# Youssef-Harby/flac-raster

Measured on AMD Instinct MI355X. Metric: Mpixels/sec encode (create-streaming) + bbox-extract ms, 1/2/4/8 GPU; bit-exact vs ref, higher is better.
Workload: dtype int16; 1 GPU; C4 create-streaming encode (band 1, device-resident); raster=40000x40000x4 int16, tile_size=512, tiles=6241, tiles_rank0=6241, blocksize=4096, compression_level=5, parallelism=single GPU (no exchange), compressed_bytes_rank0=3134407161, compressed_bytes_total=3134407161

## Files before the change

flac_raster_amd/csrc/frs_encode.hip:

```cpp

#include <type_traits>

#include <cstring>
#include <unistd.h>

#include "frs_internal.h"
#include "frs_frame_header.h"

namespace frs {

template <int DT> struct Elem;
template <> struct Elem<FRS_DT_U8> { using T = uint8_t; static constexpr bool is_float = false; };
template <> struct Elem<FRS_DT_U16> { using T = uint16_t; static constexpr bool is_float = false; };
template <> struct Elem<FRS_DT_I16> { using T = int16_t; static constexpr bool is_float = false; };
template <> struct Elem<FRS_DT_I32> { using T = int32_t; static constexpr bool is_float = false; };
template <> struct Elem<FRS_DT_U32> { using T = uint32_t; static constexpr bool is_float = false; };
template <> struct Elem<FRS_DT_F32> { using T = float; static constexpr bool is_float = true; };
template <> struct Elem<FRS_DT_F64> { using T = double; static constexpr bool is_float = true; };

__device__ inline int64_t f2key(double v) {
    int64_t b = __double_as_longlong(v);
    return b >= 0 ? b : (b ^ 0x7FFFFFFFFFFFFFFFll);
}
__host__ __device__ inline double key2f(int64_t k) {
    int64_t b = k >= 0 ? k : (k ^ 0x7FFFFFFFFFFFFFFFll);
    double d;
    memcpy(&d, &b, 8);
    return d;
}

template <int DT> __device__ inline int64_t elem_key(typename Elem<DT>::T v) {
    if constexpr (Elem<DT>::is_float) return f2key((double)v);
    else return (int64_t)v;
}

template <int DT> __device__ inline int32_t spatial_norm(typename Elem<DT>::T x) {
    if constexpr (DT == FRS_DT_U8) return cast_f64_i32_x86((double)__fdiv_rn(__fsub_rn((float)x, 127.5f), 127.5f));
    else if constexpr (DT == FRS_DT_U16) return cast_f64_i32_x86((double)__fdiv_rn(__fsub_rn((float)x, 32767.5f), 32767.5f));
    else if constexpr (DT == FRS_DT_I16) return cast_f64_i32_x86((double)__fdiv_rn((float)x, 32767.0f));
    else if constexpr (DT == FRS_DT_I32) return cast_f64_i32_x86((double)__fdiv_rn((float)x, 2147483647.0f));
    else if constexpr (DT == FRS_DT_F32) return cast_f64_i32_x86((double)fminf(fmaxf(x, -1.0f), 1.0f));
    else return 0;
}

template <int DT> struct Normalizer {
    using T = typename Elem<DT>::T;
    T mn;
    double den;
    double rinv;
    double scale;
    int has_range;
    int bps16;
    int spatial;
    int fastdiv;
    __device__ inline int32_t operator()(T x) const {
        if (spatial) return spatial_norm<DT>(x);
        if constexpr (DT == FRS_DT_F32) {
            float v = x * 8388607.0f;
            return cast_f64_i32_x86((double)v);
        } else if constexpr (DT == FRS_DT_F64) {
            return cast_f64_i32_x86(x * 8388607.0);
        } else {
            if (!has_range) return 0;
            T d = (T)((int64_t)x - (int64_t)mn);
            double v;
            if (fastdiv) {
                const double a = 2.0 * (double)d;
                const double q0 = a * rinv;
                v = fma(fma(-q0, den, a), rinv, q0) - 1.0;
            } else {
                v = (2.0 * (double)d) / den - 1.0;
            }
            v = v * scale;
            int32_t c = cast_f64_i32_x86(v);
            return bps16 ? (int32_t)(int16_t)c : c;
        }
    }
};

template <int DT> __device__ inline Normalizer<DT> make_norm(const TileNorm &tn, int scale_bits, int norm_mode) {
    Normalizer<DT> nz;
    nz.spatial = norm_mode == 1;
    using T = typename Elem<DT>::T;
    if constexpr (!Elem<DT>::is_float) nz.mn = (T)tn.imin;
    else nz.mn = (T)0;
    nz.den = tn.den;
    nz.rinv = tn.rinv;
    nz.fastdiv = tn.mode == kNormLut || tn.mode == kNormFastDiv;
    nz.scale = scale_bits == 16 ? 32767.0 : 8388607.0;
    nz.has_range = tn.has_range;
// ... 1277 lines not shown
            __syncthreads();
            uint64_t wbase = 0;
            for (int k = 0; k < wv; k++) wbase += wtot[k];
            const uint64_t excl = wbase + incl - my;
            uint64_t total = 0;
            for (int k = 0; k < kEncThreads / 64; k++) total += wtot[k];
            sub_end = pos + (uint64_t)pbits * (1 << po) + total;
            if (sub_end > (uint64_t)kWords * 32 - 64) {
                if (tid == 0) atomicOr(error_flag, 2);
                return;
            }
            uint64_t run = excl;
            __shared__ uint64_t pstart[1 << kMaxPo];
            for (int i = max(i_beg, o); i < i_end; i++) {
                const int32_t r32 = (int32_t)resid(Lc, type == 2, o, i);
                const uint32_t u = ((uint32_t)r32 << 1) ^ (uint32_t)(r32 >> 31);
                const int p = i / ps;
                const int k = rc.k[p];
                const uint32_t q = u >> k;
                const int first_of_p = p == 0 ? o : p * ps;
                if (i == first_of_p) pstart[p] = run;
                const uint64_t at = pos + (uint64_t)pbits * (p + 1) + run + q;
                const uint32_t low = k ? (u & ((1u << k) - 1u)) : 0u;
                put_bits(S.bits, at, (1u << k) | low, k + 1);
                run += 1 + (uint64_t)k + q;
            }
            __syncthreads();
            for (int p = tid; p < (1 << po); p += kEncThreads)
                put_bits(S.bits, pos + (uint64_t)pbits * p + pstart[p], rc.k[p], pbits);
            }
        }
        __syncthreads();
        {
            const uint64_t full = sub_end >> 5;
            if ((int64_t)(w0 + full) + 2 > P.slot_words) {
                if (tid == 0) atomicOr(error_flag, 1);
                return;
            }
            for (uint64_t i = tid; i < full; i += kEncThreads) slot[w0 + i] = __builtin_bswap32(S.bits[i]);
            __syncthreads();
            const uint32_t keep = S.bits[full];
            __syncthreads();
            for (int i = tid; i < kWords; i += kEncThreads) S.bits[i] = 0;
            __syncthreads();
            if (tid == 0) S.bits[0] = keep;
            __syncthreads();
            w0 += (int64_t)full;
            fb = sub_end - (full << 5);
        }
    }
    const uint64_t bits_total = (uint64_t)w0 * 32 + fb;
    const uint64_t bytes = (bits_total + 7) >> 3;
    if (fb && tid == 0) slot[w0] = __builtin_bswap32(S.bits[0]);
    if (tid == 0) frame_bytes[si] = (int64_t)bytes + 2;
}

__constant__ uint16_t c_crc16[256];
__constant__ uint16_t c_xpow8[40];

__device__ inline uint32_t gf_mulmod(uint32_t a, uint32_t b) {
    uint32_t r = 0;
#pragma unroll
    for (int i = 15; i >= 0; i--) {
        r <<= 1;
        if (r & 0x10000u) r ^= 0x18005u;
        if ((b >> i) & 1u) r ^= a;
    }
    return r;
}

__device__ inline uint32_t xpow8(uint64_t m) {
    uint32_t r = 1;
    int j = 0;
    while (m) {
        if (m & 1) r = gf_mulmod(r, c_xpow8[j]);
        m >>= 1;
        j++;
    }
    return r;
}

constexpr int kFrameWordsV3 = 2176;
constexpr int kXpowBytes = kFrameWordsV3 * 4 + 64;
__constant__ uint16_t c_crc16x8[16][256];
__device__ uint16_t g_xpow_bytes[kXpowBytes];
__device__ uint16_t g_xpow_8k[32];
__device__ inline uint32_t xpow_bytes(int64_t m) {
    if (m < kXpowBytes) return g_xpow_bytes[m];
    if (m < 32 * 8192) return gf_mulmod(g_xpow_bytes[m & 8191], g_xpow_8k[m >> 13]);
    return xpow8((uint64_t)m);
}

__device__ inline uint32_t wg_crc16(const uint8_t *src, int64_t L, const uint16_t (*T)[256], uint32_t *wc) {
    const uint32_t *sw = reinterpret_cast<const uint32_t *>(src);
    const int64_t nw = L >> 2;
    const int64_t ch = (nw + 255) / 256;
    const int64_t w0 = min(nw, (int64_t)threadIdx.x * ch), w1 = min(nw, w0 + ch);
    uint32_t c = 0;
    for (int64_t i = w0; i < w1; i++) {
        const uint32_t v = sw[i];
        c = (uint32_t)T[3][((c >> 8) ^ v) & 0xFF] ^ T[2][((c & 0xFF) ^ (v >> 8)) & 0xFF] ^ T[1][(v >> 16) & 0xFF] ^
            T[0][v >> 24];
    }
    int64_t end = w1 << 2;
    const bool last = (nw == 0) ? threadIdx.x == 0 : (w1 == nw && w1 > w0);
    if (last) {
        for (int64_t i = nw << 2; i < L; i++) c = ((c << 8) & 0xFFFFu) ^ T[0][((c >> 8) ^ src[i]) & 0xFF];
        end = L;
    }
    const int64_t m = L - end;
    if (c && m > 0) c = gf_mulmod(c, xpow_bytes(m));
    for (int o = 32; o > 0; o >>= 1) c ^= __shfl_xor(c, o);
    if ((threadIdx.x & 63) == 0) wc[threadIdx.x >> 6] = c;
    __syncthreads();
    return wc[0] ^ wc[1] ^ wc[2] ^ wc[3];
}

__device__ inline void wg_load_crc_tables(uint16_t (*T)[256]) {
    for (int i = threadIdx.x; i < 1024; i += blockDim.x) (&T[0][0])[i] = (&c_crc16x8[0][0])[i];
    __syncthreads();
}

__global__ void __launch_bounds__(256) k_compact(const uint32_t *slots, int slot_words, const int64_t *frame_bytes,
                                                const int64_t *frame_off, int64_t nframes, uint8_t *arena) {
    __shared__ uint16_t T[4][256];
    __shared__ uint32_t wc[4];
    const int64_t f = blockIdx.x;
    if (f >= nframes) return;
    wg_load_crc_tables(T);
    const uint32_t *sw = slots + (size_t)f * slot_words;
    const uint8_t *src = reinterpret_cast<const uint8_t *>(sw);
    const int64_t S = frame_bytes[f];
    const int64_t L = S - 2;
    uint8_t *dst = arena + frame_off[f];
    const int h = (int)((4 - (reinterpret_cast<uintptr_t>(dst) & 3)) & 3);
    const int64_t hb = min((int64_t)h, L);
    if ((int64_t)threadIdx.x < hb) dst[threadIdx.x] = src[threadIdx.x];
    const int64_t nbw = (L - hb) >> 2;
    uint32_t *dw = reinterpret_cast<uint32_t *>(dst + hb);
    const int sh = (int)(hb & 3);
    const int64_t swords = slot_words;
    for (int64_t k = threadIdx.x; k < nbw; k += 256) {
        const int64_t sbyte = hb + 4 * k, si = sbyte >> 2;
        const uint32_t lo = sw[si], hi = (sh && si + 1 < swords) ? sw[si + 1] : 0u;
        dw[k] = __builtin_amdgcn_alignbyte(hi, lo, (uint32_t)sh);
    }
    for (int64_t i = hb + 4 * nbw + threadIdx.x; i < L; i += 256) dst[i] = src[i];
    const uint32_t crc = wg_crc16(src, L, T, wc);
    if (threadIdx.x == 0) {
        dst[L] = (uint8_t)(crc >> 8);
        dst[L + 1] = (uint8_t)crc;
    }
}

__global__ void __launch_bounds__(256) k_seal_partial(uint32_t *slots, int slot_words, const int64_t *frame_bytes,
                                                     int64_t nlist) {
    __shared__ uint16_t T[4][256];
    __shared__ uint32_t wc[4];
    const int64_t si = blockIdx.x;
    if (si >= nlist) return;
    wg_load_crc_tables(T);
    uint8_t *src = reinterpret_cast<uint8_t *>(slots + (size_t)si * slot_words);
    const int64_t L = frame_bytes[si] - 2;
    const uint32_t crc = wg_crc16(src, L, T, wc);
    if (threadIdx.x == 0) {
        src[L] = (uint8_t)(crc >> 8);
        src[L + 1] = (uint8_t)crc;
    }
}
// ... 737 lines not shown
    v += bfly_partner64<32>(v);
    return ((uint64_t)uni((uint32_t)(v >> 32)) << 32) | uni((uint32_t)v);
}
__device__ inline uint32_t dpp_wave_or_u32(uint32_t v) {
    v |= bfly_partner<1>(v);
    v |= bfly_partner<2>(v);
    v |= bfly_partner<4>(v);
    v |= bfly_partner<8>(v);
    v |= bfly_partner<16>(v);
    v |= bfly_partner<32>(v);
    return uni(v);
}
__device__ inline uint32_t dpp_wave_max_u32(uint32_t v) {
    v = max(v, bfly_partner<1>(v));
    v = max(v, bfly_partner<2>(v));
    v = max(v, bfly_partner<4>(v));
    v = max(v, bfly_partner<8>(v));
    v = max(v, bfly_partner<16>(v));
    v = max(v, bfly_partner<32>(v));
    return uni(v);
}
__device__ inline uint32_t dpp_wave_xor_u32(uint32_t v) {
    v ^= bfly_partner<1>(v);
    v ^= bfly_partner<2>(v);
    v ^= bfly_partner<4>(v);
    v ^= bfly_partner<8>(v);
    v ^= bfly_partner<16>(v);
    v ^= bfly_partner<32>(v);
    return uni(v);
}
__device__ inline uint32_t dpp_incl_scan_u32(uint32_t v) {
    v += (uint32_t)__builtin_amdgcn_update_dpp(0, (int)v, 0x111, 0xF, 0xF, false);
    v += (uint32_t)__builtin_amdgcn_update_dpp(0, (int)v, 0x112, 0xF, 0xF, false);
    v += (uint32_t)__builtin_amdgcn_update_dpp(0, (int)v, 0x114, 0xF, 0xF, false);
    v += (uint32_t)__builtin_amdgcn_update_dpp(0, (int)v, 0x118, 0xF, 0xF, false);
    v += (uint32_t)__builtin_amdgcn_update_dpp(0, (int)v, 0x142, 0xA, 0xF, false);
    v += (uint32_t)__builtin_amdgcn_update_dpp(0, (int)v, 0x143, 0xC, 0xF, false);
    return v;
}
__device__ inline uint32_t dpp_wave_shr1(uint32_t v) {
    return (uint32_t)__builtin_amdgcn_update_dpp(0, (int)v, 0x138, 0xF, 0xF, false);
}

typedef short v2s16 __attribute__((ext_vector_type(2)));
__device__ inline int32_t dot2(uint32_t a, uint32_t b, int32_t c) {
    return __builtin_amdgcn_sdot2(__builtin_bit_cast(v2s16, a), __builtin_bit_cast(v2s16, b), c, false);
}
__device__ inline uint32_t pack2(int32_t lo, int32_t hi) { return ((uint32_t)lo & 0xFFFFu) | ((uint32_t)hi << 16); }

__device__ inline int32_t dot2_z(uint32_t a, uint32_t b) {
    int32_t d;
    asm("v_dot2_i32_i16 %0, %1, %2, 0" : "=v"(d) : "v"(a), "v"(b));
    return d;
}

__device__ inline void residual_pair(const uint32_t *E, const uint32_t *C, int shift, int m, int32_t &re, int32_t &ro) {
    const int b = 4 + m;
    const uint32_t o0 = __builtin_amdgcn_perm(E[b], E[b - 1], 0x05040302u);
    const uint32_t o1 = __builtin_amdgcn_perm(E[b - 1], E[b - 2], 0x05040302u);
    const uint32_t o2 = __builtin_amdgcn_perm(E[b - 2], E[b - 3], 0x05040302u);
    const uint32_t o3 = __builtin_amdgcn_perm(E[b - 3], E[b - 4], 0x05040302u);
    int32_t se = dot2_z(E[b - 1], C[0]);
    int32_t so = dot2_z(o0, C[0]);
    se = dot2(E[b - 2], C[1], se);
    so = dot2(o1, C[1], so);
    se = dot2(E[b - 3], C[2], se);
    so = dot2(o2, C[2], so);
    se = dot2(E[b - 4], C[3], se);
    so = dot2(o3, C[3], so);
    const uint32_t v = E[b];
    re = (int32_t)(int16_t)(v & 0xFFFFu) - (se >> shift);
    ro = ((int32_t)v >> 16) - (so >> shift);
}

constexpr uint64_t kFlagAgg = 1ull << 62, kFlagIncl = 2ull << 62, kValMask = (1ull << 62) - 1;


constexpr int kXpowHi = (kXpowBytes + 63) / 64;
constexpr int kBufWordsV3 = kFrameWordsV3 + 64;
constexpr int kSubWords = kFrameWordsV3 + 4;
struct EncV3Shared {
    uint32_t bits[4][kBufWordsV3];
    int16_t lut[kLutCap];
    uint16_t crc8x[16][256];
    uint16_t xlo[64];
    uint16_t xhi[kXpowHi];
    uint8_t crc8[256];
    int ticket[2];
    int want[2];
    int lut_tile;
};
static_assert(offsetof(EncV3Shared, lut) + sizeof(int16_t) * kLutCap <= 65536, "LUT beyond 64 KiB of LDS");

struct FbMap {
    uint32_t c, magic, k;
    __device__ inline uint32_t col(uint32_t w) const { return __umul24(w, magic) >> 20; }
    __device__ inline uint32_t operator()(uint32_t w) const {
        return (uint32_t)__mul24((int)col(w), -(int)k) + (w << 6);
    }
};
__device__ inline FbMap fb_map(uint32_t words) {
    const uint32_t c = max(1u, (words + 63) >> 6);
    return FbMap{c, ((1u << 20) + c - 1) / c, 64 * c - 1};
}
__device__ inline void fb_fold(uint32_t *buf, const FbMap &M, int lane) {
    uint32_t *ovr = buf + (M.c << 6) + lane;
    const uint32_t v = *ovr;
    *ovr = 0;
    if (lane < 63 && v) atomicOr(buf + lane + 1, v);
}

__device__ inline void lds_put_bits2(uint32_t *buf, const FbMap &M, uint32_t pos, uint32_t val, int nbits) {
    const uint32_t wi = pos >> 5;
    const uint64_t v = (uint64_t)val << (64 - (int)(pos & 31) - nbits);
    atomicOr(&buf[M(wi)], (uint32_t)(v >> 32));
    atomicOr(&buf[M(wi + 1)], (uint32_t)v);
}

__device__ inline void reg_fence(uint32_t *E) {
#pragma unroll
    for (int m = 0; m < 36; m++) asm volatile("" : "+v"(E[m]));
}

__device__ inline uint32_t sad_u32(uint32_t a, uint32_t b, uint32_t c) {
    uint32_t d;
    asm("v_sad_u32 %0, %1, %2, %3" : "=v"(d) : "v"(a), "v"(b), "v"(c));
    return d;
}

__device__ inline void lds_put_left(uint32_t *buf, const FbMap &M, int nk4, uint32_t pos, uint32_t codeL) {
    const uint32_t hi = __builtin_amdgcn_alignbit(0u, codeL, pos);
    const uint32_t lo = __builtin_amdgcn_alignbit(codeL, 0u, pos);
    const uint32_t wi = pos >> 5;
    uint32_t *p = reinterpret_cast<uint32_t *>(reinterpret_cast<char *>(buf) + (wi << 8) +
                                               __mul24((int)M.col(wi), nk4));
    atomicOr(p, hi);
    atomicOr(p + 64, lo);
}

__device__ inline void lut_gather_pairs(const uint32_t *w, const int16_t *lut, int32_t imin, uint32_t *out) {
    const uint32_t lb = (uint32_t)reinterpret_cast<uintptr_t>(lut);
    const uint32_t c16 = (lb - 2u * (uint32_t)imin) & 0xFFFFu, cc = c16 | (c16 << 16), two = 0x00020002u;
    const char *lds0 = reinterpret_cast<const char *>(lut) - lb;
#pragma unroll
    for (int m = 0; m < 32; m++) {
        uint32_t a;
        asm("v_pk_mad_u16 %0, %1, %2, %3" : "=v"(a) : "v"(w[m]), "v"(two), "v"(cc));
        const uint32_t lo = *reinterpret_cast<const uint16_t *>(lds0 + (a & 0xFFFFu));
        const uint32_t hi = *reinterpret_cast<const uint16_t *>(lds0 + (a >> 16));
        out[m] = lo | (hi << 16);
    }
}

__device__ inline uint32_t zigzag(int32_t r) { return ((uint32_t)r << 1) ^ (uint32_t)(r >> 31); }

struct PendingFrame {
    int64_t f = -1;
    uint64_t fbytes = 0;
    bool ok = true;
    FbMap map{1, 1u << 20, 63};
};

__device__ __forceinline__ void resolve_and_store(const EncodeParams &P, PendingFrame &pf, uint32_t *fbuf, uint8_t *arena,
                                         int64_t arena_cap, int64_t *frame_off, uint64_t *status, int *err, int lane) {
    const int64_t f = pf.f;
    const uint64_t fbytes = pf.fbytes;
    const bool ok = pf.ok;
    const bool l0 = lane == 0;
    uint64_t prefix = 0;
// ... 330 lines not shown
                uint32_t k = (g[c] < 2 || prod == 0) ? 0u : 32u - (uint32_t)__builtin_clz(prod);
                k = min(k, 14u);
                Kp[c] |= k << (4 * (5 - po));
                V[c][5 - po] = 4 + (1 + k) * ns + ((2 * g[c]) >> k) - (ns >> 1);
            }
        }
#pragma unroll
        for (int c = 0; c < NC; c++) V[c][0] += bfly_partner<2>(V[c][0]);
#pragma unroll
        for (int c = 0; c < NC; c++)
#pragma unroll
            for (int i = 0; i <= 1; i++) V[c][i] += bfly_partner<4>(V[c][i]);
#pragma unroll
        for (int c = 0; c < NC; c++)
#pragma unroll
            for (int i = 0; i <= 2; i++) V[c][i] += bfly_partner<8>(V[c][i]);
#pragma unroll
        for (int c = 0; c < NC; c++)
#pragma unroll
            for (int i = 0; i <= 3; i++) V[c][i] += bfly_partner<16>(V[c][i]);
#pragma unroll
        for (int c = 0; c < NC; c++)
#pragma unroll
            for (int i = 0; i <= 4; i++) V[c][i] += bfly_partner<32>(V[c][i]);
#pragma unroll
        for (int c = 0; c < NC; c++) {
            uint32_t best_bits = 0;
            int best_i = 0;
#pragma unroll
            for (int i = 0; i < 6; i++) {
                const uint32_t bits = 6 + uni(V[c][i]);
                if (best_bits == 0 || bits < best_bits) {
                    best_bits = bits;
                    best_i = i;
                }
            }
            bb[c] = best_bits;
            bp[c] = 5 - best_i;
            bk[c] = (int)((Kp[c] >> (4 * best_i)) & 15u);
        }
    };
    auto rice = [&](uint32_t lane_sum, int order, uint32_t &best_bits, int &best_po, int &my_k) {
        if (__ballot(lane_sum >= (1u << 24)) == 0) {
            const uint32_t sm[1] = {lane_sum};
            const int od[1] = {order};
            uint32_t b1[1];
            int p1[1], k1[1];
            rice32m(std::integral_constant<int, 1>{}, sm, od, b1, p1, k1);
            best_bits = b1[0], best_po = p1[0], my_k = k1[0];
        } else {
            rice64(lane_sum, order, best_bits, best_po, my_k);
        }
    };
    rb_f = rb_l = 0;
    po_f = po_l = k_f = k_l = 0;
    if (cand_fixed && cand_lpc && __ballot(sf >= (1u << 24) || sl >= (1u << 24)) == 0) {
        uint32_t bb[2];
        int bp[2], bk[2];
        const uint32_t sm[2] = {sf, sl};
        const int od[2] = {of, ol};
        rice32m(std::integral_constant<int, 2>{}, sm, od, bb, bp, bk);
        rb_f = bb[0], po_f = bp[0], k_f = bk[0];
        rb_l = bb[1], po_l = bp[1], k_l = bk[1];
    } else {
        if (cand_fixed) rice(sf, of, rb_f, po_f, k_f);
        if (cand_lpc) rice(sl, ol, rb_l, po_l, k_l);
    }
}

constexpr int kPrivRows = 34;
constexpr uint32_t kPrivBits = kPrivRows * 32;
static_assert(kBufWordsV3 >= (kPrivRows + 1) * 64, "private rows + the spill row");
static_assert(kBufWordsV3 % 4 == 0, "b128 zeroing");

__device__ inline void zero_wave_buf(uint32_t *buf, int lane) {
    uint4 *b4 = reinterpret_cast<uint4 *>(buf);
#pragma unroll
    for (int i = 0; i < (kBufWordsV3 / 4 + 63) / 64; i++) {
        const int c = lane + 64 * i;
        if (i < kBufWordsV3 / 256 || c < kBufWordsV3 / 4) b4[c] = make_uint4(0u, 0u, 0u, 0u);
    }
}

__device__ __forceinline__ uint32_t crc16_cols(const uint32_t *fbuf, const FbMap &M, uint32_t body, const EncV3Shared &S,
                                               int lane) {
    const uint32_t nfw = body >> 2, tail = body & 3;
    const uint32_t wb = min(nfw, (uint32_t)lane * M.c), we = min(nfw, wb + M.c);
    uint32_t c = 0;
    const uint32_t *colp = fbuf + lane;
    const uint16_t(*T)[256] = S.crc8x;
    uint32_t i = wb;
    for (; i + 3 < we; i += 4, colp += 256) {
        const uint32_t w0 = colp[0], w1 = colp[64], w2 = colp[128], w3 = colp[192];
        c = (uint32_t)T[15][((c >> 8) ^ (w0 >> 24)) & 0xFF] ^ T[14][((c & 0xFF) ^ (w0 >> 16)) & 0xFF] ^
            T[13][(w0 >> 8) & 0xFF] ^ T[12][w0 & 0xFF] ^ T[11][w1 >> 24] ^ T[10][(w1 >> 16) & 0xFF] ^
            T[9][(w1 >> 8) & 0xFF] ^ T[8][w1 & 0xFF] ^ T[7][w2 >> 24] ^ T[6][(w2 >> 16) & 0xFF] ^
            T[5][(w2 >> 8) & 0xFF] ^ T[4][w2 & 0xFF] ^ T[3][w3 >> 24] ^ T[2][(w3 >> 16) & 0xFF] ^
            T[1][(w3 >> 8) & 0xFF] ^ T[0][w3 & 0xFF];
    }
    for (; i + 1 < we; i += 2, colp += 128) {
        const uint32_t w0 = colp[0], w1 = colp[64];
        c = (uint32_t)T[7][((c >> 8) ^ (w0 >> 24)) & 0xFF] ^ T[6][((c & 0xFF) ^ (w0 >> 16)) & 0xFF] ^
            T[5][(w0 >> 8) & 0xFF] ^ T[4][w0 & 0xFF] ^ T[3][w1 >> 24] ^ T[2][(w1 >> 16) & 0xFF] ^
            T[1][(w1 >> 8) & 0xFF] ^ T[0][w1 & 0xFF];
    }
    if (i < we) {
        const uint32_t word = *colp;
        c = (uint32_t)T[3][((c >> 8) ^ (word >> 24)) & 0xFF] ^ T[2][((c & 0xFF) ^ (word >> 16)) & 0xFF] ^
            T[1][(word >> 8) & 0xFF] ^ T[0][word & 0xFF];
    }
    uint32_t end = we * 4;
    if (lane == (int)M.col(nfw - 1)) {
        const uint32_t word = fbuf[M(nfw)];
        for (uint32_t b = 0; b < tail; b++) {
            const uint32_t byte = (word >> (24 - 8 * b)) & 0xFF;
            c = ((c << 8) & 0xFFFFu) ^ S.crc8x[0][((c >> 8) ^ byte) & 0xFF];
        }
        end += tail;
    }
    const uint32_t m = body - end;
    return dpp_wave_xor_u32(gf_mulmod(gf_mulmod(c, S.xlo[m & 63]), S.xhi[m >> 6]));
}

template <int DT, bool SUB = false, bool ST = false, bool WIDE = false>
__device__ __forceinline__ void encode_frame_v4(const typename Elem<DT>::T *raster, const EncodeParams &P,
                                                const TileGeom *__restrict__ tiles,
                                                const TileNorm *__restrict__ norms,
                                                const SubAnalysis *__restrict__ ana, uint8_t *arena, int64_t arena_cap,
                                                int64_t *frame_off, uint64_t *status, int *err, EncV3Shared &S,
                                                int want, int64_t f, int lane, const int32_t *ftile,
                                                PendingFrame &prev, const uint4 *hdr_tab, int hdr_n,
                                                const uint32_t *pslots, const int64_t *pbytes, int chn = 0,
                                                uint32_t *sub_slots = nullptr, int32_t *sub_bits = nullptr,
                                                int32_t *sub_est = nullptr) {
    using T = typename Elem<DT>::T;
    using Lane = std::conditional_t<WIDE, LaneWide, LanePairs>;
    uint32_t *fbuf = S.bits[uni_if<!WIDE>(threadIdx.x >> 6)];
    const int t = ftile[f];
    const TileGeom g = tiles[t];
    const bool l0 = lane == 0;
    if (!SUB && g.partial && f - g.frame_base == g.nframes - 1) {
        const int64_t si = g.partial - 1;
        const uint64_t nb = (uint64_t)pbytes[si];
        const uint32_t words = (uint32_t)((nb + 3) >> 2);
        const bool ok = words + 2 <= (uint32_t)kFrameWordsV3;
        if (!ok && l0) atomicOr(err, 2);
        const uint64_t fbytes = ok ? nb : 0;
        const FbMap M = fb_map(words + 1);
        __builtin_amdgcn_s_setprio(2);
        if (l0)
            __hip_atomic_store(&status[f], (f == 0 ? kFlagIncl : kFlagAgg) | fbytes, __ATOMIC_RELAXED,
                               __HIP_MEMORY_SCOPE_AGENT);
        if (prev.f >= 0) resolve_and_store(P, prev, fbuf, arena, arena_cap, frame_off, status, err, lane);
        if (ok) {
            const uint32_t *src = pslots + (size_t)si * P.slot_words;
            for (uint32_t w = (uint32_t)lane; w < words; w += 64) fbuf[M(w)] = __builtin_bswap32(src[w]);
        }
        __builtin_amdgcn_s_waitcnt(0xC07F);
        __builtin_amdgcn_wave_barrier();
        __builtin_amdgcn_s_setprio(0);
        prev.f = f, prev.fbytes = fbytes, prev.ok = ok, prev.map = M;
        return;
    }
    TileNorm tn = norms[t];
    if (t != want && tn.mode == kNormLut) tn.mode = kNormSlow;
    const int16_t *lut = S.lut;
    __builtin_amdgcn_s_setprio(2);
    const int64_t fk = f - g.frame_base;
    const int64_t s0 = fk * kMaxBlock;
    constexpr int n = kMaxBlock;
    const int64_t sub = SUB ? f * P.nvch + chn : f;
    const SubAnalysis A = ana[sub];
    const int w = A.wasted;
    const int sbps = 16 - w + ((ST && chn == 3) ? 1 : 0);
    const T *base = raster + (int64_t)(P.band0 + ((ST && chn >= 2) ? 0 : chn)) * P.band_stride + g.r0 * P.row_stride +
                    g.c0;

    auto load_lane = [&](Lane &Ls) __attribute__((always_inline)) {
        Chunk64<DT> ch;
        const uint32_t sl0 = (uint32_t)s0 + 64u * (uint32_t)lane;
        const uint32_t row = udiv_inv(sl0, (uint32_t)g.w, 1.0 / (double)g.w);
        const int col = (int)(sl0 - row * (uint32_t)g.w), vec = (g.w % 64) == 0 ? P.vec_ok : 0;
        ch.load(base, P.row_stride, g.w, row, col, vec, 64);
        const bool lutp = sizeof(T) == 2 && tn.mode == kNormLut && w == 0;
        auto sx = [](uint32_t v, int h) -> int32_t { return h ? ((int32_t)v >> 16) : (int32_t)(int16_t)(v & 0xFFFFu); };
        if constexpr (WIDE) {
            if (lutp) {
                uint32_t Lp[32], Rp[32];
                lut_gather_pairs(ch.w, lut, (int32_t)tn.imin, Lp);
                ch.load(base + P.band_stride, P.row_stride, g.w, row, col, vec, 64);
                lut_gather_pairs(ch.w, lut, (int32_t)tn.imin, Rp);
#pragma unroll
                for (int m = 0; m < 32; m++) {
                    Ls.X[8 + 2 * m] = sx(Lp[m], 0) - sx(Rp[m], 0);
                    Ls.X[9 + 2 * m] = sx(Lp[m], 1) - sx(Rp[m], 1);
                }
            } else {
                norm_chunk<DT>(ch, tn, lut, [&](int j, int32_t x) { Ls.X[8 + j] = x; });
                ch.load(base + P.band_stride, P.row_stride, g.w, row, col, vec, 64);
                norm_chunk<DT>(ch, tn, lut, [&](int j, int32_t x) { Ls.X[8 + j] = (Ls.X[8 + j] - x) >> w; });
            }
        } else {
            auto pairs = [&](uint32_t *dst, int sh) __attribute__((always_inline)) {
// ... 296 lines not shown
            const int sr = P.sample_rate;
            put8(0xFF);
            put8(0xF8);
            put8((uint32_t)((12 << 4) | src));
            put8((uint32_t)(4 << 1));
            const uint32_t v = (uint32_t)fk;
            if (v < 0x80) put8(v);
            else if (v < 0x800) { put8(0xC0 | (v >> 6)); put8(0x80 | (v & 0x3F)); }
            else if (v < 0x10000) { put8(0xE0 | (v >> 12)); put8(0x80 | ((v >> 6) & 0x3F)); put8(0x80 | (v & 0x3F)); }
            else if (v < 0x200000) { put8(0xF0 | (v >> 18)); put8(0x80 | ((v >> 12) & 0x3F)); put8(0x80 | ((v >> 6) & 0x3F)); put8(0x80 | (v & 0x3F)); }
            else if (v < 0x4000000) { put8(0xF8 | (v >> 24)); put8(0x80 | ((v >> 18) & 0x3F)); put8(0x80 | ((v >> 12) & 0x3F)); put8(0x80 | ((v >> 6) & 0x3F)); put8(0x80 | (v & 0x3F)); }
            else { put8(0xFC | (v >> 30)); put8(0x80 | ((v >> 24) & 0x3F)); put8(0x80 | ((v >> 18) & 0x3F)); put8(0x80 | ((v >> 12) & 0x3F)); put8(0x80 | ((v >> 6) & 0x3F)); put8(0x80 | (v & 0x3F)); }
            if (srx == 12) put8((uint32_t)(sr / 1000));
            else if (srx == 13) { put8((uint32_t)(sr >> 8) & 0xFF); put8((uint32_t)sr & 0xFF); }
            else if (srx == 14) { put8((uint32_t)((sr / 10) >> 8) & 0xFF); put8((uint32_t)(sr / 10) & 0xFF); }
            put8(c8);
        }
        const int typecode = type == 0 ? 0 : type == 1 ? 1 : type == 2 ? 8 + of : 32 + ol - 1;
        lds_put_bits2(fbuf, M, hdr_bits, (uint32_t)(typecode << 1) | (w ? 1u : 0u), 8);
        if (w) lds_put_bits2(fbuf, M, hdr_bits + 8 + (uint32_t)(w - 1), 1, 1);
        if (type == 0) lds_put_bits2(fbuf, M, pos0, xi & ((1u << sbps) - 1u), sbps);
        if (type >= 2) {
            uint32_t qq = pos0 + (uint32_t)o * sbps;
            if (type == 3) {
                lds_put_bits2(fbuf, M, qq, (uint32_t)(A.lpc_prec - 1), 4);
                lds_put_bits2(fbuf, M, qq + 4, (uint32_t)lshift & 31u, 5);
                qq += 9 + (uint32_t)o * A.lpc_prec;
            }
            lds_put_bits2(fbuf, M, qq, (uint32_t)po, 6);
        }
    }
    if (type >= 2) {
        const int i = lane & 7;
        const int32_t qi = ana[sub].q[i];
        const bool warm = lane < 8 && i < o, coef = type == 3 && lane >= 8 && lane < 16 && i < o;
        if (warm) lds_put_bits2(fbuf, M, pos0 + (uint32_t)i * sbps, xi & ((1u << sbps) - 1u), sbps);
        if (coef)
            lds_put_bits2(fbuf, M, pos0 + (uint32_t)o * sbps + 9 + (uint32_t)i * A.lpc_prec,
                          (uint32_t)qi & ((1u << A.lpc_prec) - 1u), A.lpc_prec);
    }
    __builtin_amdgcn_s_waitcnt(0xC07F);
    __builtin_amdgcn_wave_barrier();
    if (fold) {
        fb_fold(fbuf, M, lane);
        __builtin_amdgcn_s_waitcnt(0xC07F);
        __builtin_amdgcn_wave_barrier();
    }
    if constexpr (SUB) {
        if (ok) {
            uint32_t *dst = sub_slots + (size_t)sub * kSubWords;
            const uint32_t nw = (end_bits + 31) >> 5;
            for (uint32_t wi = (uint32_t)lane; wi < nw; wi += 64) dst[wi] = fbuf[M(wi)];
            for (uint32_t i = 0; i < M.c; i++) fbuf[(i << 6) | (uint32_t)lane] = 0;
        } else {
            zero_wave_buf(fbuf, lane);
        }
        if (l0) sub_bits[sub] = ok ? (int32_t)end_bits : -1;
        if (l0 && sub_est) sub_est[sub] = (int32_t)best;
        (void)fbytes;
        return;
    }
    if (ok) {
        const uint32_t crc = crc16_cols(fbuf, M, body, S, lane);
        if (l0) lds_put_bits2(fbuf, M, body << 3, crc, 16);
        __builtin_amdgcn_s_waitcnt(0xC07F);
        __builtin_amdgcn_wave_barrier();
    }
    prev.f = f, prev.fbytes = fbytes, prev.ok = ok, prev.map = M;
}

template <int DT, bool SUB = false, bool ST = false, bool WIDE = false>
__global__ void __launch_bounds__(256, sizeof(typename Elem<DT>::T) <= 2 ? (ST ? 2 : 3) : 1) k_encode_v4(const typename Elem<DT>::T *raster, EncodeParams P,
                                                  const TileGeom *__restrict__ tiles,
                                                  const TileNorm *__restrict__ norms, const int16_t *__restrict__ luts,
                                                  const SubAnalysis *__restrict__ ana, uint8_t *arena, int64_t arena_cap,
                                                  int64_t *frame_off, uint64_t *status, int *ticket_ctr, int *err,
                                                  const int32_t *__restrict__ ftile, const uint4 *__restrict__ hdr_tab,
                                                  int hdr_n, const uint32_t *__restrict__ pslots,
                                                  const int64_t *__restrict__ pbytes, uint32_t *sub_slots = nullptr,
                                                  int32_t *sub_bits = nullptr, int32_t *sub_est = nullptr) {
    __shared__ __attribute__((aligned(16))) EncV3Shared S;
    constexpr bool kUni = !WIDE;
    const int wave = (int)uni_if<kUni>(threadIdx.x >> 6), lane = threadIdx.x & 63;
    for (int i = threadIdx.x; i < 4096; i += blockDim.x) (&S.crc8x[0][0])[i] = (&c_crc16x8[0][0])[i];
    for (int i = threadIdx.x; i < 256; i += blockDim.x) S.crc8[i] = c_crc8[i];
    for (int i = threadIdx.x; i < 64; i += blockDim.x) S.xlo[i] = g_xpow_bytes[i];
    for (int i = threadIdx.x; i < kXpowHi; i += blockDim.x) S.xhi[i] = g_xpow_bytes[64 * i];
    for (int i = threadIdx.x; i < 4 * kBufWordsV3; i += blockDim.x) (&S.bits[0][0])[i] = 0;
    if (threadIdx.x == 0) S.lut_tile = -1;
    PendingFrame prev;
    uint32_t *fbuf = S.bits[wave];
    int it = 0;
    while (true) {
        const int sl = it & 1;
        it++;
        constexpr int kUpfSt = WIDE ? 1 : 3;
        const int upf = ST ? kUpfSt : P.nch;
        const int64_t nunits = SUB ? P.nframes * upf : P.nframes;
        if (threadIdx.x == 0) {
            const int tk = atomicAdd(ticket_ctr, 1);
            S.ticket[sl] = tk;
            const int64_t u0 = (int64_t)tk * 4;
            S.want[sl] = (u0 < nunits) ? ftile[SUB ? u0 / upf : u0] : -1;
        }
        __syncthreads();
        const int64_t fbase = (int64_t)(int)uni_if<kUni>((uint32_t)S.ticket[sl]) * 4;
        if (fbase >= nunits) break;
        const int want = (int)uni_if<kUni>((uint32_t)S.want[sl]);
        if (want != (int)uni_if<kUni>((uint32_t)S.lut_tile)) {
            const TileNorm tw = norms[want];
            if (tw.mode == kNormLut) {
                const int64_t R = min(tw.imax - tw.imin, (int64_t)kLutCap - 1);
                const int16_t *src = luts + (int64_t)want * kLutCap;
                for (int64_t d = threadIdx.x; d <= R; d += blockDim.x) S.lut[d] = src[d];
            }
            __syncthreads();
            if (threadIdx.x == 0) S.lut_tile = want;
        }
        if constexpr (SUB) {
            const int64_t v = fbase + wave;
            if (v < nunits) {
                const int64_t f = v / upf;
                const int chn = WIDE ? 3 : (int)(v - f * upf);
                const TileGeom g = tiles[ftile[f]];
                if (!(g.partial && f - g.frame_base == g.nframes - 1))
                    encode_frame_v4<DT, true, ST, WIDE>(raster, P, tiles, norms, ana, arena, arena_cap, frame_off,
                                                        status, err, S, want, f, lane, ftile, prev, hdr_tab, hdr_n,
                                                        pslots, pbytes, chn, sub_slots, sub_bits, sub_est);
            }
        } else {
            const int64_t f = fbase + wave;
            if (f < nunits)
                encode_frame_v4<DT>(raster, P, tiles, norms, ana, arena, arena_cap, frame_off, status, err, S, want, f,
                                    lane, ftile, prev, hdr_tab, hdr_n, pslots, pbytes);
        }
    }
    if constexpr (!SUB)
        if (prev.f >= 0) resolve_and_store(P, prev, fbuf, arena, arena_cap, frame_off, status, err, lane);
}


__device__ inline int mc_frame_header(uint8_t *h, uint32_t v, int chcode, int sr) {
    return frame_header(h, 4096, sr, 16, chcode, v, c_crc8);
}

__device__ inline int st_pick(const int32_t *est4) {
    const uint32_t e0 = (uint32_t)est4[0], e1 = (uint32_t)est4[1], e2 = (uint32_t)est4[2], e3 = (uint32_t)est4[3];
    const uint32_t bits[4] = {e0 + e1, e0 + e3, e1 + e3, e2 + e3};
    int ca = 0;
    for (int k = 1; k < 4; k++)
        if (bits[k] < bits[ca]) ca = k;
    return ca;
}
__device__ inline void st_subs(int ca, int &a, int &b) {
    a = ca == 2 ? 3 : ca == 3 ? 2 : 0;
    b = ca == 0 ? 1 : ca == 2 ? 1 : 3;
}

__global__ void k_mc_frame_bytes(const EncodeParams P, const TileGeom *tiles, const int32_t *ftile,
                                 const int32_t *sub_bits, const int64_t *pbytes, int64_t *frame_bytes, int *err,
                                 const int32_t *sub_est = nullptr, int8_t *pick = nullptr) {
    const int64_t f = (int64_t)blockIdx.x * blockDim.x + threadIdx.x;
    if (f >= P.nframes) return;
    const TileGeom g = tiles[ftile[f]];
    const int64_t fk = f - g.frame_base;
    if (g.partial && fk == g.nframes - 1) {
        frame_bytes[f] = pbytes[g.partial - 1];
        return;
    }
    uint8_t h[16];
// ... 98 lines not shown
                c = ((c << 8) & 0xFFFFu) ^ T[0][((c >> 8) ^ byte) & 0xFF];
            }
            end = B;
        }
        const int64_t m = B - end;
        if (c && m > 0) c = gf_mulmod(c, xpow_bytes(m));
        for (int d = 32; d > 0; d >>= 1) c ^= __shfl_xor(c, d);
        if ((tid & 63) == 0) wc[tid >> 6] = c;
        __syncthreads();
        const uint32_t crc = wc[0] ^ wc[1] ^ wc[2] ^ wc[3];
        if (tid == 0) {
            W[B >> 2] |= ((crc >> 8) & 0xFF) << (24 - 8 * (B & 3));
            W[(B + 1) >> 2] |= (crc & 0xFF) << (24 - 8 * ((B + 1) & 3));
        }
        __syncthreads();
    }
    const int64_t S = B + 2;
    const int hh = (int)((4 - (reinterpret_cast<uintptr_t>(dst) & 3)) & 3);
    const int64_t hbytes = min((int64_t)hh, S);
    auto byte_at = [&](int64_t i) -> uint8_t { return (uint8_t)(W[i >> 2] >> (24 - 8 * (i & 3))); };
    if (tid < hbytes) dst[tid] = byte_at(tid);
    const int64_t nbw = (S - hbytes) >> 2;
    uint32_t *dw = reinterpret_cast<uint32_t *>(dst + hbytes);
    const int sh = (int)(hbytes & 3);
    for (int64_t k = tid; k < nbw; k += 256) {
        const int64_t si = (hbytes + 4 * k) >> 2;
        const uint32_t lo = __builtin_bswap32(W[si]), hi = sh ? __builtin_bswap32(W[si + 1]) : 0u;
        dw[k] = __builtin_amdgcn_alignbyte(hi, lo, (uint32_t)sh);
    }
    for (int64_t i = hbytes + 4 * nbw + tid; i < S; i += 256) dst[i] = byte_at(i);
}

__global__ void k_fast_finish(const int64_t *frame_off, const uint64_t *status, const TileGeom *tiles,
                              const TileNorm *norms, const int *err_flag, int ntiles, int64_t nframes, int64_t *pack) {
    int t = blockIdx.x * blockDim.x + threadIdx.x;
    double *mm = reinterpret_cast<double *>(pack + ntiles + 1);
    if (t < ntiles) {
        pack[t] = frame_off[tiles[t].frame_base];
        mm[2 * t] = norms[t].dmin;
        mm[2 * t + 1] = norms[t].dmax;
    }
    if (t == ntiles) {
        pack[t] = (int64_t)(status[nframes - 1] & kValMask);
        pack[3 * (int64_t)ntiles + 1] = *err_flag;
    }
}

static bool g_tables_ready[64];

static const uint8_t *host_crc8() {
    static uint8_t t[256];
    static const bool ready = (crc8_table(t), true);
    (void)ready;
    return t;
}

static int upload_tables(frs_ctx *ctx) {
    if (g_tables_ready[ctx->device]) return FRS_OK;
    const uint8_t *t8 = host_crc8();
    uint16_t t16[256];
    for (int i = 0; i < 256; i++) {
        uint16_t d = (uint16_t)(i << 8);
        for (int k = 0; k < 8; k++) d = (d & 0x8000) ? (uint16_t)((d << 1) ^ 0x8005) : (uint16_t)(d << 1);
        t16[i] = d;
    }
    uint16_t xp[40];
    auto mulmod = [](uint32_t a, uint32_t b) {
        uint32_t r = 0;
        for (int i = 15; i >= 0; i--) {
            r <<= 1;
            if (r & 0x10000u) r ^= 0x18005u;
            if ((b >> i) & 1u) r ^= a;
        }
        return r;
    };
    uint32_t v = 0x100;
    for (int j = 0; j < 40; j++) {
        xp[j] = (uint16_t)v;
        v = mulmod(v, v);
    }
    FRS_HIP(hipMemcpyToSymbolAsync(HIP_SYMBOL(c_crc8), t8, 256, 0, hipMemcpyHostToDevice, ctx->stream));
    FRS_HIP(hipMemcpyToSymbolAsync(HIP_SYMBOL(c_crc16), t16, sizeof(t16), 0, hipMemcpyHostToDevice, ctx->stream));
    FRS_HIP(hipMemcpyToSymbolAsync(HIP_SYMBOL(c_xpow8), xp, sizeof(xp), 0, hipMemcpyHostToDevice, ctx->stream));
    static uint16_t t4[16][256];
    static uint16_t xb[kXpowBytes];
    for (int i = 0; i < 256; i++) t4[0][i] = t16[i];
    for (int k = 1; k < 16; k++)
        for (int i = 0; i < 256; i++) {
            const uint16_t c = t4[k - 1][i];
            t4[k][i] = (uint16_t)(((c << 8) & 0xFFFF) ^ t16[c >> 8]);
        }
    uint32_t pw = 1;
    for (int m = 0; m < kXpowBytes; m++) {
        xb[m] = (uint16_t)pw;
        pw = mulmod(pw, 0x100);
    }
    FRS_HIP(hipMemcpyToSymbolAsync(HIP_SYMBOL(c_crc16x8), t4, sizeof(t4), 0, hipMemcpyHostToDevice, ctx->stream));
    FRS_HIP(hipMemcpyToSymbolAsync(HIP_SYMBOL(g_xpow_bytes), xb, sizeof(xb), 0, hipMemcpyHostToDevice, ctx->stream));
    static uint16_t x8k[32];
    uint32_t x8192 = 1;
    for (int m = 0; m < 8192; m++) x8192 = mulmod(x8192, 0x100);
    uint32_t q = 1;
    for (int j = 0; j < 32; j++) {
        x8k[j] = (uint16_t)q;
        q = mulmod(q, x8192);
    }
    FRS_HIP(hipMemcpyToSymbolAsync(HIP_SYMBOL(g_xpow_8k), x8k, sizeof(x8k), 0, hipMemcpyHostToDevice, ctx->stream));
    FRS_HIP(hipStreamSynchronize(ctx->stream));
    g_tables_ready[ctx->device] = true;
    return FRS_OK;
}

int dtype_size(int dt) {
    switch (dt) {
    case FRS_DT_U8: return 1;
    case FRS_DT_U16:
    case FRS_DT_I16: return 2;
    case FRS_DT_I32:
    case FRS_DT_U32:
    case FRS_DT_F32: return 4;
    case FRS_DT_F64: return 8;
    default: return 0;
    }
}

static int stream_bps_of(const frs_encode_desc *d) {
    return (d->norm_mode == 0 && d->bits_per_sample == 16) ? 16 : 32;
}

static int qlp_precision_for(int bps, int blocksize) {
    if (bps < 16) return (2 + bps / 2) > 5 ? 2 + bps / 2 : 5;
    if (bps == 16) {
        if (blocksize <= 192) return 7;
        if (blocksize <= 384) return 8;
        if (blocksize <= 576) return 9;
        if (blocksize <= 1152) return 10;
        if (blocksize <= 2304) return 11;
        if (blocksize <= 4608) return 12;
        return 13;
    }
    if (blocksize <= 384) return 13;
    if (blocksize <= 1152) return 14;
    return 15;
}

static int64_t slot_words_for(const frs_encode_desc *d) {
    const int64_t bps = stream_bps_of(d);
    const int64_t bits = 16 * 8 + (int64_t)d->nbands * (16 + 32 + (int64_t)d->blocksize * bps) +
                         (d->nbands == 2 ? (int64_t)d->blocksize : 0) + 64;
    return (bits + 31) / 32 + (int64_t)d->blocksize / 8 + 64;
}

static void build_tiles(const frs_encode_desc *d, std::vector<TileGeom> &tiles, int64_t &nframes) {
    const int64_t tcols = (d->width + d->tile_w - 1) / d->tile_w;
    nframes = 0;
    tiles.clear();
    for (int64_t ti = d->tile_begin; ti < d->tile_end; ti++) {
        TileGeom g;
        const int64_t tr = ti / tcols, tc = ti % tcols;
        g.r0 = tr * d->tile_h;
        g.c0 = tc * d->tile_w;
        g.h = (int32_t)std::min<int64_t>(d->tile_h, d->height - g.r0);
        g.w = (int32_t)std::min<int64_t>(d->tile_w, d->width - g.c0);
        const int64_t px = (int64_t)g.h * g.w;
        g.nframes = (int32_t)((px + d->blocksize - 1) / d->blocksize);
        g.frame_base = nframes;
        g.partial = 0;
        nframes += g.nframes;
        tiles.push_back(g);
    }
}

int64_t arena_bound(const frs_encode_desc *d) {
    std::vector<TileGeom> tiles;
    int64_t nframes;
    build_tiles(d, tiles, nframes);
    return nframes * (slot_words_for(d) * 4) + 64;
}

constexpr int kFastDeclined = 1000;

static std::vector<float> tukey_window(int L, float p) {
    std::vector<float> win(L, 1.0f);
    const int Np = (int)(p / 2.0f * (float)L) - 1;
    if (Np > 0)
        for (int k = 0; k <= Np; k++) {
            win[k] = (float)(0.5f - 0.5f * cos(M_PI * k / Np));
            win[L - Np - 1 + k] = (float)(0.5f - 0.5f * cos(M_PI * (k + Np) / Np));
        }
    return win;
// ... 599 lines not shown
```

Measured before the change: 319,900 Mpixels/s.

## Replace table-driven column CRC16 with carry-less polynomial folding

The per-lane CRC16 over frame-buffer columns no longer uses 16 sliced lookup tables held in LDS. It now XOR-folds the words into 17 accumulators using the polynomial's structure, then reduces them to a residue, and fixes the tail with a biased power-of-x factor from a new precomputed table that includes negative exponents. This removes 8 KiB of LDS tables, the per-block copy that fills them, and the bank-conflicted table lookups. In exchange it adds ALU work to reduce the residue, and bit-exactness now depends on the biased offset arithmetic and on padding past the end of the body being handled correctly.

```diff
diff --git a/flac_raster_amd/csrc/frs_crc16_fold.h b/flac_raster_amd/csrc/frs_crc16_fold.h
--- /dev/null
+++ b/flac_raster_amd/csrc/frs_crc16_fold.h
@@ -0,0 +1,163 @@
+#pragma once
+#include <stdint.h>
+
+#ifndef FRS_HD
+#ifdef __HIPCC__
+#define FRS_HD __host__ __device__
+#else
+#define FRS_HD
+#endif
+#endif
+#ifdef __HIPCC__
+#define FRS_UNROLL _Pragma("unroll")
+#else
+#define FRS_UNROLL
+#endif
+
+namespace frs {
+
+constexpr int kCrcFoldSpan = 45;
+constexpr int kCrcAcc = 17;
+
+FRS_HD inline void crc16_fold_word(uint32_t *A, int k, uint32_t w) {
+    const int q = k / 15, r = k % 15;
+    A[r] ^= w;
+    if (q) A[r + q] ^= w;
+}
+
+FRS_HD inline void crc16_fold_carry(uint32_t *A) {
+    A[0] ^= A[15];
+    A[1] ^= A[15] ^ A[16];
+    A[2] ^= A[16];
+    A[15] = A[16] = 0;
+}
+
+template <int N, int S>
+FRS_HD inline uint32_t crc16_shr_word(const uint32_t *V, int j) {
+    constexpr int ws = S / 32, bs = S % 32;
+    const int i = j + ws;
+    const uint32_t lo = i < N ? V[i] : 0u;
+    if constexpr (bs == 0) {
+        return lo;
+    } else {
+        const uint32_t hi = i + 1 < N ? V[i + 1] : 0u;
+        return (lo >> bs) | (hi << (32 - bs));
+    }
+}
+
+template <int N, int M, int B, int T>
+FRS_HD inline void crc16_fold_bits(const uint32_t *V, uint32_t *R) {
+    static_assert(B == 15 * T && T < 32 && 32 * M >= B, "fold point and multiplier");
+    FRS_UNROLL
+    for (int j = 0; j < M; j++) {
+        uint32_t lo = 0;
+        if (32 * (j + 1) <= B) lo = V[j];
+        else if (32 * j < B) lo = V[j] & ((1u << (B - 32 * j)) - 1u);
+        uint32_t h2 = crc16_shr_word<N, B - T>(V, j);
+        if (j == 0) h2 &= ~((1u << T) - 1u);
+        R[j] = lo ^ crc16_shr_word<N, B>(V, j) ^ h2;
+    }
+}
+
+FRS_HD inline uint32_t crc16_residue(const uint32_t *A) {
+    uint32_t a[8], b[5], c[3], d[2], e[2], f[1], g[1], h[1];
+    crc16_fold_bits<15, 8, 240, 16>(A, a);
+    crc16_fold_bits<8, 5, 120, 8>(a, b);
+    crc16_fold_bits<5, 3, 60, 4>(b, c);
+    crc16_fold_bits<3, 2, 30, 2>(c, d);
+    crc16_fold_bits<2, 2, 15, 1>(d, e);
+    crc16_fold_bits<2, 1, 15, 1>(e, f);
+    crc16_fold_bits<1, 1, 15, 1>(f, g);
+    crc16_fold_bits<1, 1, 15, 1>(g, h);
+    return h[0];
+}
+
+FRS_HD inline uint32_t crc16_parity(uint32_t v) { return (uint32_t)__builtin_popcount(v) & 1u; }
+
+FRS_HD inline uint32_t crc16_join(uint32_t res, uint32_t par) {
+    return res ^ (crc16_parity(res) != par ? 0x8003u : 0u);
+}
+
+FRS_HD inline uint32_t crc16_finish(uint32_t res, uint32_t x) {
+    uint32_t t[1] = {(res << 2) ^ (res << 1)}, r[1];
+    crc16_fold_bits<1, 1, 15, 1>(t, r);
+    return crc16_join(r[0], crc16_parity(x));
+}
+
+FRS_HD inline uint32_t crc16_reduce64(uint64_t v) {
+    uint32_t a[2] = {(uint32_t)v, (uint32_t)(v >> 32)}, b[2], c[2], d[1];
+    crc16_fold_bits<2, 2, 30, 2>(a, b);
+    crc16_fold_bits<2, 2, 15, 1>(b, c);
+    crc16_fold_bits<1, 1, 15, 1>(c, d);
+    return crc16_join(d[0], crc16_parity(a[0] ^ a[1]));
+}
+
+FRS_HD inline uint32_t crc16_tail(uint32_t crc, uint32_t word, int t) {
+    if (t == 0) return crc;
+    return crc16_reduce64(((uint64_t)crc << (8 * t)) ^ ((uint64_t)(word >> (32 - 8 * t)) << 16));
+}
+
+template <int N, int G = 1>
+FRS_HD inline uint32_t crc16_column(const uint32_t *p, int stride, int c) {
+    static_assert(N <= kCrcFoldSpan, "one fold pass");
+    uint32_t A[kCrcAcc] = {0}, x = 0;
+    FRS_UNROLL
+    for (int i = 0; i < N; i++) {
+        if (i % G == 0 && i >= c) break;
+        const uint32_t w = p[i * stride];
+        x ^= w;
+        crc16_fold_word(A, N - 1 - i, w);
+    }
+    crc16_fold_carry(A);
+    return crc16_finish(crc16_residue(A), x);
+}
+
+FRS_HD inline uint32_t crc16_words(const uint32_t *p, long stride, long n) {
+    uint32_t A[kCrcAcc] = {0}, x = 0;
+    const long nb = n > kCrcFoldSpan ? (n - kCrcFoldSpan + 14) / 15 : 0, t = n - 15 * nb;
+    FRS_UNROLL
+    for (int k = kCrcFoldSpan - 1; k >= 0; k--) {
+        if (k < t) {
+            const uint32_t w = p[(t - 1 - k) * stride];
+            x ^= w;
+            crc16_fold_word(A, k, w);
+        }
+    }
+    crc16_fold_carry(A);
+    const uint32_t *q = p + t * stride;
+    for (long b = 0; b < nb; b++, q += 15 * stride) {
+        const uint32_t carry = A[14];
+        FRS_UNROLL
+        for (int r = 14; r >= 1; r--) {
+            const uint32_t w = q[(14 - r) * stride];
+            x ^= w;
+            A[r] ^= A[r - 1] ^ w;
+        }
+        const uint32_t w = q[14 * stride];
+        x ^= w;
+        A[0] ^= carry ^ w;
+        A[1] ^= carry;
+    }
+    return crc16_finish(crc16_residue(A), x);
+}
+
+FRS_HD inline uint32_t crc16_mulmod(uint32_t a, uint32_t b) {
+    uint32_t r = 0;
+    for (int i = 15; i >= 0; i--) {
+        r <<= 1;
+        if (r & 0x10000u) r ^= 0x18005u;
+        if ((b >> i) & 1u) r ^= a;
+    }
+    return r;
+}
+
+FRS_HD inline uint32_t crc16_xpow(long e) {
+    uint32_t r = 1, s = e < 0 ? 0xC002u : 2u;
+    for (unsigned long m = e < 0 ? 0ul - (unsigned long)e : (unsigned long)e; m; m >>= 1) {
+        if (m & 1) r = crc16_mulmod(r, s);
+        s = crc16_mulmod(s, s);
+    }
+    return r;
+}
+
+}
diff --git a/flac_raster_amd/csrc/frs_encode.hip b/flac_raster_amd/csrc/frs_encode.hip
--- a/flac_raster_amd/csrc/frs_encode.hip
+++ b/flac_raster_amd/csrc/frs_encode.hip
@@ -6,6 +6,7 @@
 
 #include "frs_internal.h"
 #include "frs_frame_header.h"
+#include "frs_crc16_fold.h"
 
 namespace frs {
 
@@ -1449,9 +1450,10 @@
 
 constexpr int kFrameWordsV3 = 2176;
 constexpr int kXpowBytes = kFrameWordsV3 * 4 + 64;
-__constant__ uint16_t c_crc16x8[16][256];
+__constant__ uint16_t c_crc16x8[4][256];
 __device__ uint16_t g_xpow_bytes[kXpowBytes];
 __device__ uint16_t g_xpow_8k[32];
+__device__ uint16_t g_xpow_hi[(kXpowBytes + 63) / 64 + 3];
 __device__ inline uint32_t xpow_bytes(int64_t m) {
     if (m < kXpowBytes) return g_xpow_bytes[m];
     if (m < 32 * 8192) return gf_mulmod(g_xpow_bytes[m & 8191], g_xpow_8k[m >> 13]);
@@ -2355,9 +2357,8 @@
 struct EncV3Shared {
     uint32_t bits[4][kBufWordsV3];
     int16_t lut[kLutCap];
-    uint16_t crc8x[16][256];
     uint16_t xlo[64];
-    uint16_t xhi[kXpowHi];
+    uint16_t xhi[kXpowHi + 3];
     uint8_t crc8[256];
     int ticket[2];
     int want[2];
@@ -2854,43 +2855,16 @@
     }
 }
 
+constexpr int kCrcRows = kFrameWordsV3 / 64;
+constexpr int kCrcBias = 192;
+static_assert(kFrameWordsV3 % 64 == 0 && kCrcRows <= frs::kCrcFoldSpan && kCrcBias % 64 == 0 && kCrcBias >= 4 * kCrcRows,
+              "column CRC");
+static_assert(kCrcRows * 64 <= kBufWordsV3 && sizeof(g_xpow_hi) == sizeof(uint16_t) * (kXpowHi + 3),
+              "the rows read (in groups of 8, below kCrcRows) are the buffer's; the factor table");
 __device__ __forceinline__ uint32_t crc16_cols(const uint32_t *fbuf, const FbMap &M, uint32_t body, const EncV3Shared &S,
                                                int lane) {
-    const uint32_t nfw = body >> 2, tail = body & 3;
-    const uint32_t wb = min(nfw, (uint32_t)lane * M.c), we = min(nfw, wb + M.c);
-    uint32_t c = 0;
-    const uint32_t *colp = fbuf + lane;
-    const uint16_t(*T)[256] = S.crc8x;
-    uint32_t i = wb;
-    for (; i + 3 < we; i += 4, colp += 256) {
-        const uint32_t w0 = colp[0], w1 = colp[64], w2 = colp[128], w3 = colp[192];
-        c = (uint32_t)T[15][((c >> 8) ^ (w0 >> 24)) & 0xFF] ^ T[14][((c & 0xFF) ^ (w0 >> 16)) & 0xFF] ^
-            T[13][(w0 >> 8) & 0xFF] ^ T[12][w0 & 0xFF] ^ T[11][w1 >> 24] ^ T[10][(w1 >> 16) & 0xFF] ^
-            T[9][(w1 >> 8) & 0xFF] ^ T[8][w1 & 0xFF] ^ T[7][w2 >> 24] ^ T[6][(w2 >> 16) & 0xFF] ^
-            T[5][(w2 >> 8) & 0xFF] ^ T[4][w2 & 0xFF] ^ T[3][w3 >> 24] ^ T[2][(w3 >> 16) & 0xFF] ^
-            T[1][(w3 >> 8) & 0xFF] ^ T[0][w3 & 0xFF];
-    }
-    for (; i + 1 < we; i += 2, colp += 128) {
-        const uint32_t w0 = colp[0], w1 = colp[64];
-        c = (uint32_t)T[7][((c >> 8) ^ (w0 >> 24)) & 0xFF] ^ T[6][((c & 0xFF) ^ (w0 >> 16)) & 0xFF] ^
-            T[5][(w0 >> 8) & 0xFF] ^ T[4][w0 & 0xFF] ^ T[3][w1 >> 24] ^ T[2][(w1 >> 16) & 0xFF] ^
-            T[1][(w1 >> 8) & 0xFF] ^ T[0][w1 & 0xFF];
-    }
-    if (i < we) {
-        const uint32_t word = *colp;
-        c = (uint32_t)T[3][((c >> 8) ^ (word >> 24)) & 0xFF] ^ T[2][((c & 0xFF) ^ (word >> 16)) & 0xFF] ^
-            T[1][(word >> 8) & 0xFF] ^ T[0][word & 0xFF];
-    }
-    uint32_t end = we * 4;
-    if (lane == (int)M.col(nfw - 1)) {
-        const uint32_t word = fbuf[M(nfw)];
-        for (uint32_t b = 0; b < tail; b++) {
-            const uint32_t byte = (word >> (24 - 8 * b)) & 0xFF;
-            c = ((c << 8) & 0xFFFFu) ^ S.crc8x[0][((c >> 8) ^ byte) & 0xFF];
-        }
-        end += tail;
-    }
-    const uint32_t m = body - end;
+    const uint32_t c = frs::crc16_column<kCrcRows, 8>(fbuf + lane, 64, (int)M.c);
+    const int m = max(0, (int)body + (kCrcBias - 4 * kCrcRows) - 4 * (int)M.c * lane);
     return dpp_wave_xor_u32(gf_mulmod(gf_mulmod(c, S.xlo[m & 63]), S.xhi[m >> 6]));
 }
 
@@ -3353,10 +3327,9 @@
     __shared__ __attribute__((aligned(16))) EncV3Shared S;
     constexpr bool kUni = !WIDE;
     const int wave = (int)uni_if<kUni>(threadIdx.x >> 6), lane = threadIdx.x & 63;
-    for (int i = threadIdx.x; i < 4096; i += blockDim.x) (&S.crc8x[0][0])[i] = (&c_crc16x8[0][0])[i];
     for (int i = threadIdx.x; i < 256; i += blockDim.x) S.crc8[i] = c_crc8[i];
     for (int i = threadIdx.x; i < 64; i += blockDim.x) S.xlo[i] = g_xpow_bytes[i];
-    for (int i = threadIdx.x; i < kXpowHi; i += blockDim.x) S.xhi[i] = g_xpow_bytes[64 * i];
+    for (int i = threadIdx.x; i < kXpowHi + 3; i += blockDim.x) S.xhi[i] = g_xpow_hi[i];
     for (int i = threadIdx.x; i < 4 * kBufWordsV3; i += blockDim.x) (&S.bits[0][0])[i] = 0;
     if (threadIdx.x == 0) S.lut_tile = -1;
     PendingFrame prev;
@@ -3621,10 +3594,10 @@
     FRS_HIP(hipMemcpyToSymbolAsync(HIP_SYMBOL(c_crc8), t8, 256, 0, hipMemcpyHostToDevice, ctx->stream));
     FRS_HIP(hipMemcpyToSymbolAsync(HIP_SYMBOL(c_crc16), t16, sizeof(t16), 0, hipMemcpyHostToDevice, ctx->stream));
     FRS_HIP(hipMemcpyToSymbolAsync(HIP_SYMBOL(c_xpow8), xp, sizeof(xp), 0, hipMemcpyHostToDevice, ctx->stream));
-    static uint16_t t4[16][256];
+    static uint16_t t4[4][256];
     static uint16_t xb[kXpowBytes];
     for (int i = 0; i < 256; i++) t4[0][i] = t16[i];
-    for (int k = 1; k < 16; k++)
+    for (int k = 1; k < 4; k++)
         for (int i = 0; i < 256; i++) {
             const uint16_t c = t4[k - 1][i];
             t4[k][i] = (uint16_t)(((c << 8) & 0xFFFF) ^ t16[c >> 8]);
@@ -3645,6 +3618,9 @@
         q = mulmod(q, x8192);
     }
     FRS_HIP(hipMemcpyToSymbolAsync(HIP_SYMBOL(g_xpow_8k), x8k, sizeof(x8k), 0, hipMemcpyHostToDevice, ctx->stream));
+    static uint16_t xhi[kXpowHi + 3];
+    for (int j = 0; j < kXpowHi + 3; j++) xhi[j] = (uint16_t)frs::crc16_xpow(512L * (j - 3));
+    FRS_HIP(hipMemcpyToSymbolAsync(HIP_SYMBOL(g_xpow_hi), xhi, sizeof(xhi), 0, hipMemcpyHostToDevice, ctx->stream));
     FRS_HIP(hipStreamSynchronize(ctx->stream));
     g_tables_ready[ctx->device] = true;
     return FRS_OK;
```

Measured after the change: 345,100 Mpixels/s (median of 6 runs). +7.9%, better.
